# AsyncFlow-Sim/AsyncFlow

Hardware: AMD Instinct MI355X
Metric: simulated request-events/sec (2-server LB scenario, 10k replicas/GPU) (higher is better)
Workload: dtype f64

## Files before the change

### asyncflow_amd/_abi.py

```python

from __future__ import annotations

import ctypes as C

AF_ABI_VERSION = 7

MAX_REQUEST_CAPACITY = 65535
MAX_FIFO_CAPACITY = 1 << 20
COMM_ID_BYTES = 128
AF_OK = 0
AF_ERR_INVALID = -1
AF_ERR_NO_DEVICE = -2
DEVICE_PLAN_ONLY = -1
AF_ERR_HIP = -3
AF_ERR_CAPACITY = -4
AF_ERR_ABI = -5

DIST_CODES = {"poisson": 0, "normal": 1, "log_normal": 2, "exponential": 3, "uniform": 4}
NODE_CLIENT, NODE_LB, NODE_SERVER = 0, 1, 2
LB_CODES = {"round_robin": 0, "least_connection": 1}
STEP_CPU, STEP_IO = 0, 1
METRIC_BITS = {
    "ready_queue_len": 1,
    "event_loop_io_sleep": 2,
# ... 162 lines not shown
        ("flow_fallback", C.c_uint32),
        ("flow_fallback_tie", C.c_uint32),
        ("flow_fallback_list", C.c_uint32),
        ("flow_fallback_ring", C.c_uint32),
        ("flow_fallback_ram", C.c_uint32),
        ("flow_retried", C.c_uint32),
        ("flow_to_next_event", C.c_uint32),
        ("flow_list_entries", C.c_uint32),
        ("flow_ring_rows", C.c_uint32),
        ("flow_lds_bytes", C.c_uint32),
        ("jit_fallbacks", C.c_uint32),
        ("gather_ms", C.c_double),
        ("pregen_group", C.c_uint32),
        ("summary_overlapped", C.c_uint32),
        ("summary_beside_ms", C.c_double),
    ]


FLOW_RING_IN_HBM = 0xFFFFFFFF


class AfSummary(C.Structure):
    _fields_ = [
        ("n_scenarios", C.c_uint32),
        ("rps_buckets", C.c_uint32),
        ("hist_bins", C.c_uint32),
        ("hist_max", C.c_double),
        ("stats", C.c_void_p),
        ("rps", C.c_void_p),
        ("hist", C.c_void_p),
# ... 164 lines not shown
```

### asyncflow_amd/csrc/af_pregen.hpp

```cpp
#pragma once

#include <stdint.h>

#include "af_core.hpp"

namespace afp {

constexpr uint32_t kBatch = 8u;
constexpr uint32_t kRound = 8u;
constexpr uint32_t kChunk = kBatch * kRound;

AF_HD double unit_variate(uint64_t seed, uint32_t idx) {
    const af::U4 r = af::draw_block(seed, af::STREAM_GENERATOR, idx, 0u);
    double u = af::u53(r.x, r.y);
    if (u < 1e-15) u = 1e-15;
    return -af::af_log_unit(1.0 - u);
}

AF_HD double refine_rcp(double d, double r0) {
    const double e0 = __builtin_fma(-d, r0, 1.0);
    const double r1 = __builtin_fma(r0, e0, r0);
    const double e1 = __builtin_fma(-d, r1, 1.0);
    return __builtin_fma(r1, e1, r1);
}
// ... 131 lines not shown
    double total_time, users_mean, users_sigma, rpm, window_s;
    uint32_t users_dist, n_scen, n_draw;
    uint32_t stride;
    uint32_t group;
    const uint64_t* seeds;
    const uint32_t* scen_map;
    uint32_t n_ovr;
    const uint32_t* ovr_param;
    const uint32_t* ovr_index;
    const double* ovr_values;
    uint32_t ovr_stride;
    double* out;
    uint32_t* pre_flags;
};

#if defined(__HIPCC__)
__device__ __forceinline__ double arrival_param(const ArrivalArgs& a, uint32_t param, uint32_t scen, double dflt) {
    for (uint32_t k = 0; k < a.n_ovr; ++k)
        if (a.ovr_param[k] == param && a.ovr_index[k] == 0u) dflt = a.ovr_values[(size_t)k * a.ovr_stride + scen];
    return dflt;
}
__device__ __noinline__ double users_draw_call(uint32_t dist, double mean, double sigma, uint64_t seed, uint32_t idx) {
    return users_draw(dist, mean, sigma, seed, idx);
}

#if !defined(AF_PREGEN_PRODUCERS)
#define AF_PREGEN_PRODUCERS 15
#endif
constexpr uint32_t kProducers = AF_PREGEN_PRODUCERS;
constexpr uint32_t kGroupThreads = 64u * (1u + kProducers);
constexpr uint32_t kIdle = 0xFFFFFFFFu;
typedef double d2_t __attribute__((ext_vector_type(2)));
struct GroupLds {
    double in[2][64][kChunk + 2u];
    double sums[2][64][kChunk + 1u];
    uint64_t seed[64];
    uint32_t d0[64];
    uint32_t sums_k[2][64], sums_n[2][64];
    uint32_t k_final[64];
    uint32_t run[2];
    uint32_t window[2];
};
static_assert(kChunk == 64u, "group_produce / group_store: one wave, one scenario per pass");
__device__ __forceinline__ void group_produce(GroupLds& M, uint32_t buf, uint32_t round, uint32_t n_here, uint32_t ptid) {
    const uint32_t j = ptid & 63u;
    for (uint32_t s = (uint32_t)__builtin_amdgcn_readfirstlane((int)(ptid >> 6)); s < n_here; s += kProducers) {
        const uint32_t d0 = (uint32_t)__builtin_amdgcn_readfirstlane((int)M.d0[s]);
        if (d0 == kIdle) continue;
        const uint32_t lo = (uint32_t)__builtin_amdgcn_readfirstlane((int)(uint32_t)M.seed[s]);
        const uint32_t hi = (uint32_t)__builtin_amdgcn_readfirstlane((int)(uint32_t)(M.seed[s] >> 32));
        M.in[buf][s][j] = unit_variate(((uint64_t)hi << 32) | lo, d0 + round * kChunk + j);
    }
}
__device__ __forceinline__ void group_store(const GroupLds& M, uint32_t buf, double* rows, uint32_t stride, uint32_t n_here,
                                            uint32_t ptid) {
    const uint32_t j = ptid & 63u;
    for (uint32_t s = (uint32_t)__builtin_amdgcn_readfirstlane((int)(ptid >> 6)); s < n_here; s += kProducers) {
        const uint32_t n = (uint32_t)__builtin_amdgcn_readfirstlane((int)M.sums_n[buf][s]);
        const uint32_t k = (uint32_t)__builtin_amdgcn_readfirstlane((int)M.sums_k[buf][s]);
        if (j < n) rows[(size_t)s * stride + k + j] = M.sums[buf][s][j];
    }
}
template <bool FAST_DIV>
__device__ __forceinline__ void group_chain_round(Lane& L, GroupLds& M, uint32_t buf, uint32_t lane, double T, uint32_t n_draw) {
    const uint32_t k0 = L.k;
    d2_t cur[kBatch / 2u], nxt[kBatch / 2u];
#pragma unroll
    for (uint32_t j = 0u; j < kBatch; j += 2u) cur[j / 2u] = *(const d2_t*)&M.in[buf][lane][j];
#pragma unroll
    for (uint32_t st = 0u; st < kRound; ++st) {
        if (st + 1u < kRound) {
#pragma unroll
            for (uint32_t j = 0u; j < kBatch; j += 2u) nxt[j / 2u] = *(const d2_t*)&M.in[buf][lane][(st + 1u) * kBatch + j];
        }
        double e[kBatch], G[kBatch], S[kBatch];
#pragma unroll
        for (uint32_t j = 0u; j < kBatch; j += 2u) {
            e[j] = cur[j / 2u].x;
            e[j + 1u] = cur[j / 2u].y;
        }
        lane_sums<FAST_DIV>(L, e, G, S);
        if (L.state == LANE_RUN) {
            double* o = &M.sums[buf][lane][L.k - k0];
#pragma unroll
            for (uint32_t j = 0u; j < kBatch; ++j) o[j] = S[j];
            if (lane_usual(L, G, T, n_draw)) lane_commit(L, G, S);
            else lane_slow(L, G, S, T, n_draw, nullptr, true);
        }
#pragma unroll
        for (uint32_t j = 0u; j < kBatch / 2u; ++j) cur[j] = nxt[j];
    }
    M.sums_k[buf][lane] = k0;
    M.sums_n[buf][lane] = L.k - k0;
    if (L.state != LANE_RUN) M.d0[lane] = kIdle;
}
__global__ void __launch_bounds__(kGroupThreads) af_arrival_groups(const ArrivalArgs a) {
    extern __shared__ __attribute__((aligned(16))) unsigned char group_smem[];
    GroupLds& M = *reinterpret_cast<GroupLds*>(group_smem);
    const uint32_t tid = threadIdx.x, lane = tid & 63u;
    const bool chain = tid < 64u;
    const uint32_t ptid = tid - 64u;
    const uint32_t slot0 = blockIdx.x * a.group;
    const uint32_t n_here = a.n_scen - slot0 < a.group ? a.n_scen - slot0 : a.group;
    const double T = a.total_time;
    double* rows = a.out + (size_t)slot0 * a.stride;
    const bool valid = chain && lane < n_here;
    const uint32_t slot = slot0 + (valid ? lane : 0u);
    const uint32_t scen = a.scen_map ? a.scen_map[slot] : slot;
    const uint64_t seed = a.seeds[scen];
    double users_mean = 0.0, users_sigma = 0.0, window_s = 0.0, rps_per_user = 0.0;
    Lane L;
    lane_init(L);
    L.state = LANE_DONE;
    if (chain) {
        users_mean = arrival_param(a, af::PARAM_GEN_USERS_MEAN, scen, a.users_mean);
        users_sigma = arrival_param(a, af::PARAM_GEN_USERS_SIGMA, scen, a.users_sigma);
        window_s = arrival_param(a, af::PARAM_GEN_WINDOW, scen, a.window_s);
        rps_per_user = arrival_param(a, af::PARAM_GEN_RPM_MEAN, scen, a.rpm) / 60.0;
        if (valid) L.state = LANE_WAIT;
        M.seed[lane] = seed;
        __builtin_amdgcn_s_setprio(3);
    }
    for (uint32_t w = 0u;; ++w) {
        if (chain) {
            if (L.state == LANE_WAIT)
                window_start(L, T, window_s, rps_per_user,
                             [&](uint32_t idx) { return users_draw_call(a.users_dist, users_mean, users_sigma, seed, idx); });
            M.d0[lane] = L.state == LANE_RUN ? L.draws : kIdle;
            const bool any_run = __any(L.state == LANE_RUN), any_left = __any(L.state != LANE_DONE);
            if (lane == 0u) M.window[w & 1u] = any_run ? 2u : any_left ? 1u : 0u;
        }
        __syncthreads();
        const uint32_t what = M.window[w & 1u];
        if (what == 0u) break;
        if (what == 1u) continue;
        if (!chain) group_produce(M, 0u, 0u, n_here, ptid);
        const bool fast = chain ? !__any(L.state == LANE_RUN && !L.fast_div) : true;
        __syncthreads();
        uint32_t r = 0u;
        for (;;) {
            const uint32_t b = r & 1u;
            if (chain) {
                if (fast) group_chain_round<true>(L, M, b, lane, T, a.n_draw);
                else group_chain_round<false>(L, M, b, lane, T, a.n_draw);
                const bool any_run = __any(L.state == LANE_RUN);
                if (lane == 0u) M.run[b] = any_run ? 1u : 0u;
            } else {
                group_produce(M, b ^ 1u, r + 1u, n_here, ptid);
                if (r > 0u) group_store(M, b ^ 1u, rows, a.stride, n_here, ptid);
            }
            __syncthreads();
            ++r;
            if (M.run[b] == 0u) break;
        }
        if (!chain) group_store(M, (r - 1u) & 1u, rows, a.stride, n_here, ptid);
    }
    if (chain) {
        M.k_final[lane] = L.k;
        if (valid) a.pre_flags[slot] = L.flags;
    }
    __syncthreads();
    for (uint32_t s = 0u; s < n_here; ++s) {
        double* o = rows + (size_t)s * a.stride;
        for (uint32_t i = M.k_final[s] + tid; i < a.n_draw; i += kGroupThreads) o[i] = af::AF_INF;
    }
}
#endif


}
```

### asyncflow_amd/csrc/engine.hip

```cpp
#include <hip/hip_runtime.h>
#include <dlfcn.h>

#include <algorithm>
#include <chrono>
#include <cmath>
#include <cstdio>
#include <cstring>
#include <string>
#include <vector>

#include "../../include/asyncflow_hip.h"
#include "af_core.hpp"
#include "af_flow_host.hpp"
#include "af_plan_pack.hpp"
#include "af_pregen.hpp"
#include "af_summary.hpp"
#include "af_pooled.hpp"
#include "af_series_windows.hpp"
#include "af_windowed.hpp"
#include "af_quantiles.hpp"

#define LDS_AS __attribute__((address_space(3)))

namespace {
// ... 245 lines not shown
        v += dpp<0x111, 0xF>(v);
        v += dpp<0x112, 0xF>(v);
        v += dpp<0x114, 0xF>(v);
        v += dpp<0x118, 0xF>(v);
        v += dpp<0x142, 0xA>(v);
        v += dpp<0x143, 0xC>(v);
        return v;
    }
    static __device__ __forceinline__ uint32_t mbcnt(uint64_t m) {
        return __builtin_amdgcn_mbcnt_hi((uint32_t)(m >> 32), __builtin_amdgcn_mbcnt_lo((uint32_t)m, 0u));
    }
    static __device__ __forceinline__ unsigned long long clock() { return __builtin_amdgcn_s_memtime(); }
};

constexpr uint32_t kDoneWords = 16u;
static __device__ __forceinline__ void signal_scenario_done(const uint32_t* counter_block, uint32_t sc) {
    if (counter_block == nullptr) return;
    const uint64_t* sig = reinterpret_cast<const uint64_t*>(counter_block + kDoneWords);
    uint32_t* flags = reinterpret_cast<uint32_t*>(sig[0]);
    if (flags != nullptr) WaveHip::signal_done(flags + sc, reinterpret_cast<uint32_t*>(sig[1]));
}

#ifndef AF_FLOW_WPE
#define AF_FLOW_WPE 4
#endif
#endif
#ifndef AF_JIT
template <uint32_t IPL, uint32_t FEAT>
__global__ void __launch_bounds__(64) __attribute__((amdgpu_waves_per_eu((FEAT & aff::FEAT_GENSRV) ? 3 : AF_FLOW_WPE))) af_flow_kernel(const aff::FlowArgs a) {
    extern __shared__ __attribute__((aligned(16))) unsigned char smem[];
// ... 280 lines not shown
        for (uint32_t i = k + l; i < a.n_draw; i += G) out[i] = af::AF_INF;
        if (l == 0u) a.pre_flags[slot] = flags;
    }
}


static uint32_t pregen_group_width(uint32_t n) {
    uint32_t group = (n + 255u) / 256u < 64u ? (n + 255u) / 256u : 64u;
    if (const char* env = std::getenv("AF_PREGEN_GROUP")) {
        const int v = std::atoi(env);
        if (v >= 1 && v <= 64) group = (uint32_t)v;
    }
    return group;
}

static int launch_pregen_arrivals(const KArgs& a, uint32_t n, uint32_t stride, bool uniform_load, hipStream_t stream,
                                  bool grouped = false, uint32_t* group_out = nullptr) {
    if (grouped) {
        afp::ArrivalArgs g{};
        g.total_time = a.total_time;
        g.users_mean = a.gen_users_mean;
        g.users_sigma = a.gen_users_sigma;
        g.rpm = a.gen_rpm_mean;
        g.window_s = a.gen_window_s;
        g.users_dist = a.gen_users_dist;
        g.n_scen = n;
        g.n_draw = a.n_draw;
        g.stride = stride;
        g.group = pregen_group_width(n);
        if (group_out) *group_out = g.group;
        g.seeds = a.seeds;
        g.scen_map = a.scen_map;
        g.n_ovr = a.n_ovr;
        g.ovr_param = a.ovr_param;
        g.ovr_index = a.ovr_index;
        g.ovr_values = a.ovr_values;
        g.ovr_stride = a.ovr_stride;
        g.out = a.draws;
        g.pre_flags = a.pre_flags;
        if (hipFuncSetAttribute(reinterpret_cast<const void*>(afp::af_arrival_groups), hipFuncAttributeMaxDynamicSharedMemorySize,
                                (int)sizeof(afp::GroupLds)) != hipSuccess)
            return 1;
        hipLaunchKernelGGL(afp::af_arrival_groups, dim3((n + g.group - 1u) / g.group), dim3(afp::kGroupThreads),
                           sizeof(afp::GroupLds), stream, g);
        return 0;
    }
    double best = 1e300;
    uint32_t best_s = 4u;
    for (uint32_t s : {4u, 5u, 8u}) {
        const double waves = std::ceil((double)n / (double)s);
        if (s != 4u && (!uniform_load || waves / 1024.0 < 1.9)) continue;
        const double cost = std::ceil(waves / 1024.0) * (4.06 * (double)s + 8.0);
        if (cost < best - 1e-9) {
            best = cost;
            best_s = s;
        }
    }
    bool rows = true;
    if (const char* env = std::getenv("AF_PREGEN_SCEN_PER_WAVE")) {
        const uint32_t v = (uint32_t)std::atoi(env);
// ... 131 lines not shown
    double* d_draws = nullptr;
    size_t draws_cap = 0;
    uint32_t* d_pre_flags = nullptr;
    size_t pre_flags_cap = 0;
    uint64_t* d_tie = nullptr;
    size_t tie_cap = 0;
    uint32_t* d_n_shared = nullptr;
    uint32_t* d_map = nullptr;
    size_t map_cap = 0;
    uint32_t* d_order = nullptr;
    size_t order_cap = 0;
    const af_summary_t* fused_sum = nullptr;
    const af_outputs_t* fused_out = nullptr;
    hipStream_t stream2 = nullptr;
    hipEvent_t ev_s0 = nullptr, ev_s1 = nullptr;
    bool fused_done = false;
    uint32_t* d_done_flags = nullptr;
    size_t done_flags_cap = 0;
    uint32_t* h_done_count = nullptr;
    uint32_t* d_done_count = nullptr;
    uint32_t* d_retry = nullptr;
    size_t retry_cap = 0;
    unsigned char* d_pool = nullptr;
    size_t pool_cap = 0;
    int wait_value_ok = -1;
    uint64_t done_ptrs[2] = {0, 0};
    bool shared_instants_likely = false;
    hipModule_t jit_module = nullptr;
    hipFunction_t jit_lean = nullptr, jit_order3 = nullptr, jit_order2 = nullptr;
    std::string jit_spec;
// ... 874 lines not shown
    };
    a.n_draw = n_draw;
    a.n_shared = e->d_n_shared;
    a.scen_map = nullptr;
    a.draw_slot = nullptr;
    a.draws_by_lane = 0u;

    double ms_pregen = 0.0, ms_kernel = 0.0, ms_flow = 0.0;
    uint32_t kl = 0, waves = 0, lds_bytes = 0, n_chunks = 0, n_rerun = 0, n_jit = 0, n_jit_miss = 0;
    uint32_t fused_first = 0u;
    uint32_t fb_total[5] = {0, 0, 0, 0, 0}, flow_scen = 0;
    uint32_t flow_retried = 0, flow_to_next = 0;
    size_t draw_bytes = 0;
    uint32_t pregen_group = 0;
    bool lds_state = false;

    aff::FlowLayout& FL = FP.FL;
    aff::FlowLayout& FL2 = FP.FL2;
    const bool flow_big = FP.big;
    const uint32_t flow_lds = FP.lds;

    const size_t tie_words = a.L.tie_words;
    const bool hetero_load = (mask & ((1u << AF_PARAM_GEN_USERS_MEAN) | (1u << AF_PARAM_GEN_RPM_MEAN))) != 0u;
    auto launch_des = [&](uint32_t count, bool faithful) -> int {
        choose_lanes(e, count, a.blob_bytes, bytes_per_lane, kl, lds_state);
        uint32_t klog = 0;
        while ((1u << klog) < kl) ++klog;
        a.n_scen = count;
        const uint64_t state_per_wave = bytes_per_lane * kl;
        waves = (count + kl - 1) / kl;
// ... 153 lines not shown
        a.pre_flags = e->d_arr_flags;
        const char* pregen_mode = std::getenv("AF_PREGEN_MODE");
        const bool force_groups = pregen_mode && std::strcmp(pregen_mode, "groups") == 0;
        const bool force_rows = pregen_mode && std::strcmp(pregen_mode, "rows") == 0;
        const bool grouped = !force_rows && a.gen_window_s > 0.0 &&
                             (force_groups || (!(mask & (1u << AF_PARAM_GEN_WINDOW)) && nc >= 3072u &&
                                               (double)n_draw * a.gen_window_s >= 512.0 * a.total_time &&
                                               (!hetero_load || load_spread_suits_groups(e, sweep, lo, nc))));
        const bool ordered = hetero_load && std::getenv("AF_FLOW_ORDER_OFF") == nullptr;
        if (ordered) {
            std::vector<uint32_t> order = heaviest_first(e, sweep, lo, nc);
            if (int rc = grow((void**)&e->d_order, e->order_cap, (size_t)nc * 4u)) return rc;
            HIP_TRY(hipMemcpyAsync(e->d_order, order.data(), (size_t)nc * 4u, hipMemcpyHostToDevice, e->stream));
            HIP_TRY(hipStreamSynchronize(e->stream));
        }
        HIP_TRY(hipEventRecord(e->ev2, e->stream));
        if (launch_pregen_arrivals(a, nc, n_draw, !hetero_load, e->stream, grouped, &pregen_group)) return fail(AF_ERR_HIP, "af_arrival_groups: LDS attribute");
        HIP_TRY(hipGetLastError());
        HIP_TRY(hipEventRecord(e->ev3, e->stream));
        aff::FlowArgs f = e->fargs;
        f.L = FL;
        f.n_scen = nc;
        f.seeds = a.seeds;
        f.n_ovr = a.n_ovr;
        f.ovr_param = a.ovr_param;
        f.ovr_index = a.ovr_index;
        f.ovr_values = a.ovr_values;
        f.ovr_stride = a.ovr_stride;
        f.arrivals = e->d_arr;
        f.n_draw = n_draw;
        f.pre_flags = e->d_arr_flags;
        if (ordered) f.scen_map = e->d_order;
        f.clock = a.clock;
        f.clock_cap = a.clock_cap;
// ... 16 lines not shown
        }
        {
            const uint32_t flow_lds_launch = spread_lds_bytes(flow_lds);
            void* kargs[] = {&f};
            const bool jit = e->flow_jit_fn != nullptr && flow_lds_launch <= 64u * 1024u &&
                             flow_jit_spec_string(e, FP, out, sweep->n_overrides != 0u) == e->flow_jit_spec;
            if (e->flow_jit_fn != nullptr && !jit) n_jit_miss += 1u;
            if (std::getenv("AF_DEBUG")) std::fprintf(stderr, "[af] flow jit spec: %s\n", flow_jit_spec_string(e, FP, out, sweep->n_overrides != 0u).c_str());
            if (std::getenv("AF_DEBUG"))
                std::fprintf(stderr, "[af] flow launch: %u scenarios, %u list entries%s, %u ring rows, %u B LDS per wave, af_flow_kernel<%u, %#x>%s%s\n", nc,
                             FL.cap, flow_big ? " (long-list instantiation)" : "", FL.ring_rows, flow_lds, FP.ipl, FP.feat,
                             FP.lean ? (FP.far ? ", lean instantiation with far edges" : ", lean instantiation") : "", jit ? ", plan-specialised" : "");
            const void* fn = jit ? nullptr : flow_kernel_for(FP.ipl, FP.feat);
            if (!jit && fn == nullptr) return fail(AF_ERR_INVALID, "no stage-parallel instantiation for this launch");
            if (!jit && flow_lds_launch > 48u * 1024u) HIP_TRY(hipFuncSetAttribute(fn, hipFuncAttributeMaxDynamicSharedMemorySize, (int)flow_lds_launch));
            uint32_t gate = 0u;
            if (e->fused_sum != nullptr && lo == 0u && nc == n && d_prof == nullptr) {
                if (e->wait_value_ok < 0) {
                    int v = 0;
                    if (hipDeviceGetAttribute(&v, hipDeviceAttributeCanUseStreamWaitValue, e->device) != hipSuccess) { (void)hipGetLastError(); v = 0; }
                    e->wait_value_ok = v;
                }
                int per_cu = 0;
                hipDeviceProp_t prop;
                HIP_TRY(hipGetDeviceProperties(&prop, e->device));
                if (jit) HIP_TRY(hipModuleOccupancyMaxActiveBlocksPerMultiprocessor(&per_cu, e->flow_jit_fn, (int)kWave, flow_lds_launch));
                else HIP_TRY(hipOccupancyMaxActiveBlocksPerMultiprocessor(&per_cu, fn, (int)kWave, flow_lds_launch));
                const uint32_t resident = (uint32_t)(per_cu > 0 ? per_cu : 0) * (uint32_t)prop.multiProcessorCount;
                const uint32_t rem = resident ? nc % resident : 0u;
                if (e->wait_value_ok > 0 && resident != 0u && nc > resident && nc <= 6u * resident && rem != 0u && rem * 4u <= resident * 3u) gate = nc - rem;
                if (std::getenv("AF_DEBUG")) std::fprintf(stderr, "[af] analyzer beside the last round: %u resident waves, gate at %u of %u scenarios\n", resident, gate, nc);
            }
            if (gate != 0u) {
                if (e->stream2 == nullptr) {
                    HIP_TRY(hipStreamCreateWithFlags(&e->stream2, hipStreamNonBlocking));
                    HIP_TRY(hipEventCreate(&e->ev_s0));
                    HIP_TRY(hipEventCreate(&e->ev_s1));
                    HIP_TRY(hipHostMalloc((void**)&e->h_done_count, 64, hipHostMallocCoherent | hipHostMallocMapped));
                    HIP_TRY(hipHostGetDevicePointer((void**)&e->d_done_count, e->h_done_count, 0));
                }
                if (int rc = grow((void**)&e->d_done_flags, e->done_flags_cap, (size_t)nc * 4u)) return rc;
                if (int rc = grow((void**)&e->d_retry, e->retry_cap, 2u * ((size_t)nc + 1u) * 4u)) return rc;
                *e->h_done_count = 0u;
                HIP_TRY(hipMemsetAsync(e->d_done_flags, 0, (size_t)nc * 4u, e->stream));
                HIP_TRY(hipMemsetAsync(e->d_retry, 0, 2u * ((size_t)nc + 1u) * 4u, e->stream));
                e->done_ptrs[0] = reinterpret_cast<uint64_t>(e->d_done_flags);
                e->done_ptrs[1] = reinterpret_cast<uint64_t>(e->d_done_count);
                HIP_TRY(hipMemcpyAsync(e->d_fb + kDoneWords, e->done_ptrs, 16u, hipMemcpyHostToDevice, e->stream));
            }
            f.n_scen = nc;
            if (jit) {
                HIP_TRY(hipModuleLaunchKernel(e->flow_jit_fn, nc, 1, 1, kWave, 1, 1, flow_lds_launch, e->stream, kargs, nullptr));
                n_jit += 1u;
            } else {
                HIP_TRY(hipLaunchKernel(fn, dim3(nc), dim3(kWave), kargs, flow_lds_launch, e->stream));
            }
            if (gate != 0u) {
                auto release_side = [&]() { *e->h_done_count = 0xFFFFFFFFu; };
                hipError_t err = hipStreamWaitValue32(e->stream2, e->d_done_count, gate, hipStreamWaitValueGte, 0xFFFFFFFFu);
                if (err == hipSuccess) err = hipEventRecord(e->ev_s0, e->stream2);
                int rc = AF_OK;
                if (err == hipSuccess) rc = launch_summary_kernels(e, e->fused_out, e->fused_sum, 0u, nc, e->stream2, e->d_done_flags, e->d_retry, nullptr, 0u);
                if (err == hipSuccess && rc == AF_OK) err = hipEventRecord(e->ev_s1, e->stream2);
                if (err != hipSuccess || rc != AF_OK) {
                    release_side();
                    (void)hipStreamSynchronize(e->stream);
                    (void)hipStreamSynchronize(e->stream2);
                    if (rc != AF_OK) return rc;
                    HIP_TRY(err);
                }
// ... 26 lines not shown
                for (uint32_t k = 0; k < aff::kProfSections; ++k) acc[k] += (double)hp[(size_t)i * aff::kProfSections + k];
            for (uint32_t k = 0; k < aff::kProfSections; ++k)
                if (!names[k] || std::strncmp(names[k], "COUNT", 5) != 0) total += acc[k];
            if (FILE* fp = std::fopen(prof_path, "a")) {
                std::fprintf(fp, "af_flow_kernel<%u, %#x> sections, %u waves, mean cycles per wave %.0f:\n", FP.ipl, FP.feat, nc, total / nc);
                for (uint32_t k = 0; k < aff::kProfSections; ++k)
                    if (names[k]) std::fprintf(fp, "  %-28s %6.2f %%  %12.0f cycles per wave\n", names[k], 100.0 * acc[k] / total, acc[k] / nc);
                std::fclose(fp);
            }
        }
        float ms_p = 0.f, ms_f = 0.f;
        HIP_TRY(hipEventElapsedTime(&ms_p, e->ev2, e->ev3));
        HIP_TRY(hipEventElapsedTime(&ms_f, e->ev3, e->ev4));
        ms_pregen += ms_p;
        ms_flow += ms_f;
        flow_scen += nc;
        for (int k = 0; k < 5; ++k) fb_total[k] += fb[k];
        if (fb[0] > 0u) {
            std::vector<uint32_t> cnt_host((size_t)nc * AF_CNT_SLOTS);
            HIP_TRY(hipMemcpy(cnt_host.data(), a.counts, cnt_host.size() * 4u, hipMemcpyDeviceToHost));
            std::vector<uint32_t> retry, rest;
            for (uint32_t i = 0; i < nc; ++i) {
                const uint32_t fl = cnt_host[(size_t)i * AF_CNT_SLOTS + AF_CNT_FLAGS];
                if (!(fl & aff::FLAG_FLOW_FALLBACK)) continue;
                if ((fl & (aff::FLOW_WHY_RAM | aff::FLOW_WHY_GEN_TIE)) || (flow_big && !FP.gen_compact)) rest.push_back(i);
                else retry.push_back(i);
            }
            if (!retry.empty()) {
                if (int rc = grow((void**)&e->d_map, e->map_cap, retry.size() * 4u)) return rc;
                HIP_TRY(hipMemcpyAsync(e->d_map, retry.data(), retry.size() * 4u, hipMemcpyHostToDevice, e->stream));
// ... 58 lines not shown
    e->stats.flow_kernel_ms = ms_flow;
    e->stats.flow_scenarios = flow_scen;
    e->stats.flow_fallback = fb_total[0];
    e->stats.flow_fallback_tie = fb_total[1];
    e->stats.flow_fallback_list = fb_total[2];
    e->stats.flow_fallback_ring = fb_total[3];
    e->stats.flow_fallback_ram = fb_total[4];
    e->stats.flow_retried = flow_retried;
    e->stats.flow_to_next_event = flow_to_next;
    e->stats.flow_list_entries = flow_scen ? FL.cap : 0u;
    e->stats.flow_ring_rows = flow_scen ? FL.ring_rows : 0u;
    e->stats.flow_lds_bytes = flow_lds;
    e->stats.jit_fallbacks = n_jit_miss;
    e->stats.pregen_group = pregen_group;
    e->stats.pregen_ms = ms_pregen;
    e->stats.h2d_ms = ms_h2d;
    e->stats.draw_bytes = draw_bytes;
    e->stats.state_bytes_per_scenario = bytes_per_lane;
    e->stats.state_in_lds = lds_state ? 1u : 0u;
    e->stats.lds_bytes_per_wave = lds_bytes;
    e->stats.waves = waves;
    e->stats.lanes_per_wave = kl;
    e->stats.chunks = n_chunks;
    e->stats.shared_instant_scenarios = n_rerun;
    e->stats.specialised_launches = n_jit;
    e->stats.request_capacity = e->request_capacity;
    e->stats.fifo_capacity = e->fifo_capacity;
    return AF_OK;
}

// ... 831 lines not shown
        delete e;
        return;
    }
    (void)hipSetDevice(e->device);
    if (e->d_blob) (void)hipFree(e->d_blob);
    if (e->d_state) (void)hipFree(e->d_state);
    if (e->d_sweep) (void)hipFree(e->d_sweep);
    if (e->ev0) (void)hipEventDestroy(e->ev0);
    if (e->ev1) (void)hipEventDestroy(e->ev1);
    if (e->ev2) (void)hipEventDestroy(e->ev2);
    if (e->ev3) (void)hipEventDestroy(e->ev3);
    if (e->ev4) (void)hipEventDestroy(e->ev4);
    if (e->ev_s0) (void)hipEventDestroy(e->ev_s0);
    if (e->ev_s1) (void)hipEventDestroy(e->ev_s1);
    if (e->stream2) (void)hipStreamDestroy(e->stream2);
    if (e->d_done_flags) (void)hipFree(e->d_done_flags);
    if (e->d_retry) (void)hipFree(e->d_retry);
    if (e->d_pool) (void)hipFree(e->d_pool);
    if (e->h_done_count) (void)hipHostFree(e->h_done_count);
    if (e->d_draws) (void)hipFree(e->d_draws);
    if (e->d_pre_flags) (void)hipFree(e->d_pre_flags);
    if (e->d_tie) (void)hipFree(e->d_tie);
    if (e->d_n_shared) (void)hipFree(e->d_n_shared);
    if (e->d_map) (void)hipFree(e->d_map);
    if (e->d_order) (void)hipFree(e->d_order);
    if (e->d_tick) (void)hipFree(e->d_tick);
    if (e->d_arr) (void)hipFree(e->d_arr);
    if (e->d_arr_flags) (void)hipFree(e->d_arr_flags);
    if (e->d_fb) (void)hipFree(e->d_fb);
    if (e->d_slot) (void)hipFree(e->d_slot);
// ... 207 lines not shown
```

### include/asyncflow_hip.h

```cpp
#ifndef ASYNCFLOW_HIP_H
#define ASYNCFLOW_HIP_H

#include <stddef.h>
#include <stdint.h>

#ifdef __cplusplus
extern "C" {
#endif

#define AF_ABI_VERSION 7

enum af_status {
    AF_OK = 0,
    AF_ERR_INVALID = -1,
    AF_ERR_NO_DEVICE = -2,
    AF_ERR_HIP = -3,
    AF_ERR_CAPACITY = -4,
    AF_ERR_ABI = -5
};

enum af_dist {
    AF_DIST_POISSON = 0,
    AF_DIST_NORMAL = 1,
    AF_DIST_LOG_NORMAL = 2,
// ... 169 lines not shown
    uint32_t flow_fallback;
    uint32_t flow_fallback_tie;
    uint32_t flow_fallback_list;
    uint32_t flow_fallback_ring;
    uint32_t flow_fallback_ram;
    uint32_t flow_retried;
    uint32_t flow_to_next_event;
    uint32_t flow_list_entries;
    uint32_t flow_ring_rows;
    uint32_t flow_lds_bytes;
    uint32_t jit_fallbacks;
    double gather_ms;
    uint32_t pregen_group;
    uint32_t summary_overlapped;
    double summary_beside_ms;
} af_stats_t;

typedef struct af_engine af_engine_t;

#define AF_DEVICE_PLAN_ONLY (-1)
int af_engine_create(const af_plan_t* plan, int device, const af_engine_options_t* opts,
                     af_engine_t** out);
int af_engine_jit_spec(af_engine_t* engine, const af_sweep_t* sweep, const af_outputs_t* out, char* buf, size_t cap);
int af_engine_set_kernels(af_engine_t* engine, const char* spec, const void* image, size_t size);

typedef struct af_summary_t {
    uint32_t n_scenarios;
    uint32_t rps_buckets;
    uint32_t hist_bins;
    double hist_max;
// ... 102 lines not shown
```

Baseline: 123.6 billion.

## Split pregen and flow launches across two streams to overlap the partial round

When the flow kernel's scenario count leaves a partial last round of resident waves, the scenarios in that remainder are now pre-generated and simulated first on the main stream. The remaining scenarios have their arrivals pre-generated on a second stream, using a smaller producer count, while that first part runs. The grouped arrival kernel is templated on producer count, and its LDS layout becomes dynamically sized by group width, so a lighter variant can run beside the flow kernel. The aim is to fill idle CUs in the tail and hide pre-generation time, at the cost of an extra stream, events, an identity map buffer, and possible contention between the concurrent kernels.

```diff
diff --git a/asyncflow_amd/_abi.py b/asyncflow_amd/_abi.py
--- a/asyncflow_amd/_abi.py
+++ b/asyncflow_amd/_abi.py
@@ -200,6 +200,9 @@
         ("pregen_group", C.c_uint32),
         ("summary_overlapped", C.c_uint32),
         ("summary_beside_ms", C.c_double),
+        ("pregen_beside_ms", C.c_double),
+        ("flow_split_first", C.c_uint32),
+        ("flow_resident", C.c_uint32),
     ]
 
 
diff --git a/asyncflow_amd/csrc/af_pregen.hpp b/asyncflow_amd/csrc/af_pregen.hpp
--- a/asyncflow_amd/csrc/af_pregen.hpp
+++ b/asyncflow_amd/csrc/af_pregen.hpp
@@ -169,6 +169,102 @@
     uint32_t* pre_flags;
 };
 
+constexpr uint32_t kIdle = 0xFFFFFFFFu;
+constexpr uint32_t kInPitch = kChunk + 2u;
+constexpr uint32_t kSumsPitch = kChunk + 1u;
+constexpr uint32_t kTailInf = 64u;
+typedef double d2_t __attribute__((vector_size(16)));
+struct GroupLds {
+    unsigned char* base;
+    uint32_t group;
+    AF_HD static uint32_t off_sums(uint32_t g) { return 2u * g * kInPitch * 8u; }
+    AF_HD static uint32_t off_seed(uint32_t g) { return off_sums(g) + 2u * g * kSumsPitch * 8u; }
+    AF_HD static uint32_t off_words(uint32_t g) { return off_seed(g) + g * 8u; }
+    AF_HD static uint32_t bytes(uint32_t g) { return (off_words(g) + (6u * g + 4u) * 4u + 15u) & ~15u; }
+    AF_HD double* in(uint32_t buf, uint32_t s) const { return reinterpret_cast<double*>(base) + (size_t)(buf * group + s) * kInPitch; }
+    AF_HD double* sums(uint32_t buf, uint32_t s) const {
+        return reinterpret_cast<double*>(base + off_sums(group)) + (size_t)(buf * group + s) * kSumsPitch;
+    }
+    AF_HD uint64_t* seed() const { return reinterpret_cast<uint64_t*>(base + off_seed(group)); }
+    AF_HD uint32_t* words() const { return reinterpret_cast<uint32_t*>(base + off_words(group)); }
+    AF_HD uint32_t* d0() const { return words(); }
+    AF_HD uint32_t* sums_k(uint32_t buf) const { return words() + (1u + buf) * group; }
+    AF_HD uint32_t* sums_n(uint32_t buf) const { return words() + (3u + buf) * group; }
+    AF_HD uint32_t* k_final() const { return words() + 5u * group; }
+    AF_HD uint32_t* run() const { return words() + 6u * group; }
+    AF_HD uint32_t* window() const { return words() + 6u * group + 2u; }
+};
+#if defined(__HIP_DEVICE_COMPILE__)
+#define AFP_UNIFORM(x) ((uint32_t)__builtin_amdgcn_readfirstlane((int)(x)))
+#else
+#define AFP_UNIFORM(x) ((uint32_t)(x))
+#endif
+static_assert(kChunk == 64u, "group_produce / group_store: one wave, one scenario per pass");
+AF_HD void group_produce(const GroupLds& M, uint32_t buf, uint32_t round, uint32_t n_here, uint32_t ptid, uint32_t producers) {
+    const uint32_t j = ptid & 63u;
+    for (uint32_t s = AFP_UNIFORM(ptid >> 6); s < n_here; s += producers) {
+        const uint32_t d0 = AFP_UNIFORM(M.d0()[s]);
+        if (d0 == kIdle) continue;
+        const uint32_t lo = AFP_UNIFORM((uint32_t)M.seed()[s]);
+        const uint32_t hi = AFP_UNIFORM((uint32_t)(M.seed()[s] >> 32));
+        M.in(buf, s)[j] = unit_variate(((uint64_t)hi << 32) | lo, d0 + round * kChunk + j);
+    }
+}
+AF_HD void group_store(const GroupLds& M, uint32_t buf, double* rows, uint32_t stride, uint32_t n_here, uint32_t ptid,
+                       uint32_t producers) {
+    const uint32_t j = ptid & 63u;
+    for (uint32_t s = AFP_UNIFORM(ptid >> 6); s < n_here; s += producers) {
+        const uint32_t n = AFP_UNIFORM(M.sums_n(buf)[s]);
+        const uint32_t k = AFP_UNIFORM(M.sums_k(buf)[s]);
+        if (j < n) rows[(size_t)s * stride + k + j] = M.sums(buf, s)[j];
+    }
+}
+template <bool FAST_DIV>
+AF_HD void group_chain_round(Lane& L, const GroupLds& M, uint32_t buf, uint32_t lane, double T, uint32_t n_draw) {
+    const uint32_t k0 = L.k;
+    const double* in = M.in(buf, lane);
+    double* sums = M.sums(buf, lane);
+    d2_t cur[kBatch / 2u], nxt[kBatch / 2u];
+#pragma unroll
+    for (uint32_t j = 0u; j < kBatch; j += 2u) cur[j / 2u] = *(const d2_t*)&in[j];
+#pragma unroll
+    for (uint32_t st = 0u; st < kRound; ++st) {
+        if (st + 1u < kRound) {
+#pragma unroll
+            for (uint32_t j = 0u; j < kBatch; j += 2u) nxt[j / 2u] = *(const d2_t*)&in[(st + 1u) * kBatch + j];
+        }
+        double e[kBatch], G[kBatch], S[kBatch];
+#pragma unroll
+        for (uint32_t j = 0u; j < kBatch; j += 2u) {
+            e[j] = cur[j / 2u][0];
+            e[j + 1u] = cur[j / 2u][1];
+        }
+        lane_sums<FAST_DIV>(L, e, G, S);
+        if (L.state == LANE_RUN) {
+            double* o = &sums[L.k - k0];
+#pragma unroll
+            for (uint32_t j = 0u; j < kBatch; ++j) o[j] = S[j];
+            if (lane_usual(L, G, T, n_draw)) lane_commit(L, G, S);
+            else lane_slow(L, G, S, T, n_draw, nullptr, true);
+        }
+        if (st + 1u < kRound) {
+#pragma unroll
+            for (uint32_t j = 0u; j < kBatch / 2u; ++j) cur[j] = nxt[j];
+        }
+    }
+    M.sums_k(buf)[lane] = k0;
+    M.sums_n(buf)[lane] = L.k - k0;
+    if (L.state != LANE_RUN) M.d0()[lane] = kIdle;
+}
+AF_HD void group_fill_tail(const GroupLds& M, double* rows, uint32_t stride, uint32_t n_draw, uint32_t n_here, uint32_t tid,
+                           uint32_t threads) {
+    const uint32_t j = tid & 63u;
+    for (uint32_t s = tid >> 6; s < n_here; s += threads >> 6) {
+        const uint32_t i = M.k_final()[s] + j;
+        if (j < kTailInf && i < n_draw) rows[(size_t)s * stride + i] = af::AF_INF;
+    }
+}
+
 #if defined(__HIPCC__)
 __device__ __forceinline__ double arrival_param(const ArrivalArgs& a, uint32_t param, uint32_t scen, double dflt) {
     for (uint32_t k = 0; k < a.n_ovr; ++k)
@@ -183,75 +279,13 @@
 #define AF_PREGEN_PRODUCERS 15
 #endif
 constexpr uint32_t kProducers = AF_PREGEN_PRODUCERS;
-constexpr uint32_t kGroupThreads = 64u * (1u + kProducers);
-constexpr uint32_t kIdle = 0xFFFFFFFFu;
-typedef double d2_t __attribute__((ext_vector_type(2)));
-struct GroupLds {
-    double in[2][64][kChunk + 2u];
-    double sums[2][64][kChunk + 1u];
-    uint64_t seed[64];
-    uint32_t d0[64];
-    uint32_t sums_k[2][64], sums_n[2][64];
-    uint32_t k_final[64];
-    uint32_t run[2];
-    uint32_t window[2];
-};
-static_assert(kChunk == 64u, "group_produce / group_store: one wave, one scenario per pass");
-__device__ __forceinline__ void group_produce(GroupLds& M, uint32_t buf, uint32_t round, uint32_t n_here, uint32_t ptid) {
-    const uint32_t j = ptid & 63u;
-    for (uint32_t s = (uint32_t)__builtin_amdgcn_readfirstlane((int)(ptid >> 6)); s < n_here; s += kProducers) {
-        const uint32_t d0 = (uint32_t)__builtin_amdgcn_readfirstlane((int)M.d0[s]);
-        if (d0 == kIdle) continue;
-        const uint32_t lo = (uint32_t)__builtin_amdgcn_readfirstlane((int)(uint32_t)M.seed[s]);
-        const uint32_t hi = (uint32_t)__builtin_amdgcn_readfirstlane((int)(uint32_t)(M.seed[s] >> 32));
-        M.in[buf][s][j] = unit_variate(((uint64_t)hi << 32) | lo, d0 + round * kChunk + j);
-    }
-}
-__device__ __forceinline__ void group_store(const GroupLds& M, uint32_t buf, double* rows, uint32_t stride, uint32_t n_here,
-                                            uint32_t ptid) {
-    const uint32_t j = ptid & 63u;
-    for (uint32_t s = (uint32_t)__builtin_amdgcn_readfirstlane((int)(ptid >> 6)); s < n_here; s += kProducers) {
-        const uint32_t n = (uint32_t)__builtin_amdgcn_readfirstlane((int)M.sums_n[buf][s]);
-        const uint32_t k = (uint32_t)__builtin_amdgcn_readfirstlane((int)M.sums_k[buf][s]);
-        if (j < n) rows[(size_t)s * stride + k + j] = M.sums[buf][s][j];
-    }
-}
-template <bool FAST_DIV>
-__device__ __forceinline__ void group_chain_round(Lane& L, GroupLds& M, uint32_t buf, uint32_t lane, double T, uint32_t n_draw) {
-    const uint32_t k0 = L.k;
-    d2_t cur[kBatch / 2u], nxt[kBatch / 2u];
-#pragma unroll
-    for (uint32_t j = 0u; j < kBatch; j += 2u) cur[j / 2u] = *(const d2_t*)&M.in[buf][lane][j];
-#pragma unroll
-    for (uint32_t st = 0u; st < kRound; ++st) {
-        if (st + 1u < kRound) {
-#pragma unroll
-            for (uint32_t j = 0u; j < kBatch; j += 2u) nxt[j / 2u] = *(const d2_t*)&M.in[buf][lane][(st + 1u) * kBatch + j];
-        }
-        double e[kBatch], G[kBatch], S[kBatch];
-#pragma unroll
-        for (uint32_t j = 0u; j < kBatch; j += 2u) {
-            e[j] = cur[j / 2u].x;
-            e[j + 1u] = cur[j / 2u].y;
-        }
-        lane_sums<FAST_DIV>(L, e, G, S);
-        if (L.state == LANE_RUN) {
-            double* o = &M.sums[buf][lane][L.k - k0];
-#pragma unroll
-            for (uint32_t j = 0u; j < kBatch; ++j) o[j] = S[j];
-            if (lane_usual(L, G, T, n_draw)) lane_commit(L, G, S);
-            else lane_slow(L, G, S, T, n_draw, nullptr, true);
-        }
-#pragma unroll
-        for (uint32_t j = 0u; j < kBatch / 2u; ++j) cur[j] = nxt[j];
-    }
-    M.sums_k[buf][lane] = k0;
-    M.sums_n[buf][lane] = L.k - k0;
-    if (L.state != LANE_RUN) M.d0[lane] = kIdle;
-}
-__global__ void __launch_bounds__(kGroupThreads) af_arrival_groups(const ArrivalArgs a) {
+constexpr uint32_t kProducersBeside = 7u;
+template <uint32_t P>
+__global__ void __launch_bounds__(64u * (1u + P)) __attribute__((amdgpu_waves_per_eu(4))) af_arrival_groups(const ArrivalArgs a) {
+    static_assert(P >= 1u && P <= 15u, "a workgroup is at most 16 waves");
+    constexpr uint32_t kGroupThreads = 64u * (1u + P);
     extern __shared__ __attribute__((aligned(16))) unsigned char group_smem[];
-    GroupLds& M = *reinterpret_cast<GroupLds*>(group_smem);
+    const GroupLds M{group_smem, a.group};
     const uint32_t tid = threadIdx.x, lane = tid & 63u;
     const bool chain = tid < 64u;
     const uint32_t ptid = tid - 64u;
@@ -272,8 +306,10 @@
         users_sigma = arrival_param(a, af::PARAM_GEN_USERS_SIGMA, scen, a.users_sigma);
         window_s = arrival_param(a, af::PARAM_GEN_WINDOW, scen, a.window_s);
         rps_per_user = arrival_param(a, af::PARAM_GEN_RPM_MEAN, scen, a.rpm) / 60.0;
-        if (valid) L.state = LANE_WAIT;
-        M.seed[lane] = seed;
+        if (valid) {
+            L.state = LANE_WAIT;
+            M.seed()[lane] = seed;
+        }
         __builtin_amdgcn_s_setprio(3);
     }
     for (uint32_t w = 0u;; ++w) {
@@ -281,44 +317,43 @@
             if (L.state == LANE_WAIT)
                 window_start(L, T, window_s, rps_per_user,
                              [&](uint32_t idx) { return users_draw_call(a.users_dist, users_mean, users_sigma, seed, idx); });
-            M.d0[lane] = L.state == LANE_RUN ? L.draws : kIdle;
+            if (valid) M.d0()[lane] = L.state == LANE_RUN ? L.draws : kIdle;
             const bool any_run = __any(L.state == LANE_RUN), any_left = __any(L.state != LANE_DONE);
-            if (lane == 0u) M.window[w & 1u] = any_run ? 2u : any_left ? 1u : 0u;
+            if (lane == 0u) M.window()[w & 1u] = any_run ? 2u : any_left ? 1u : 0u;
         }
         __syncthreads();
-        const uint32_t what = M.window[w & 1u];
+        const uint32_t what = M.window()[w & 1u];
         if (what == 0u) break;
         if (what == 1u) continue;
-        if (!chain) group_produce(M, 0u, 0u, n_here, ptid);
+        if (!chain) group_produce(M, 0u, 0u, n_here, ptid, P);
         const bool fast = chain ? !__any(L.state == LANE_RUN && !L.fast_div) : true;
         __syncthreads();
         uint32_t r = 0u;
         for (;;) {
             const uint32_t b = r & 1u;
             if (chain) {
-                if (fast) group_chain_round<true>(L, M, b, lane, T, a.n_draw);
-                else group_chain_round<false>(L, M, b, lane, T, a.n_draw);
+                if (valid) {
+                    if (fast) group_chain_round<true>(L, M, b, lane, T, a.n_draw);
+                    else group_chain_round<false>(L, M, b, lane, T, a.n_draw);
+                }
                 const bool any_run = __any(L.state == LANE_RUN);
-                if (lane == 0u) M.run[b] = any_run ? 1u : 0u;
+                if (lane == 0u) M.run()[b] = any_run ? 1u : 0u;
             } else {
-                group_produce(M, b ^ 1u, r + 1u, n_here, ptid);
-                if (r > 0u) group_store(M, b ^ 1u, rows, a.stride, n_here, ptid);
+                group_produce(M, b ^ 1u, r + 1u, n_here, ptid, P);
+                if (r > 0u) group_store(M, b ^ 1u, rows, a.stride, n_here, ptid, P);
             }
             __syncthreads();
             ++r;
-            if (M.run[b] == 0u) break;
-        }
-        if (!chain) group_store(M, (r - 1u) & 1u, rows, a.stride, n_here, ptid);
-    }
-    if (chain) {
-        M.k_final[lane] = L.k;
-        if (valid) a.pre_flags[slot] = L.flags;
+            if (M.run()[b] == 0u) break;
+        }
+        if (!chain) group_store(M, (r - 1u) & 1u, rows, a.stride, n_here, ptid, P);
+    }
+    if (valid) {
+        M.k_final()[lane] = L.k;
+        a.pre_flags[slot] = L.flags;
     }
     __syncthreads();
-    for (uint32_t s = 0u; s < n_here; ++s) {
-        double* o = rows + (size_t)s * a.stride;
-        for (uint32_t i = M.k_final[s] + tid; i < a.n_draw; i += kGroupThreads) o[i] = af::AF_INF;
-    }
+    group_fill_tail(M, rows, a.stride, a.n_draw, n_here, tid, kGroupThreads);
 }
 #endif
 
diff --git a/asyncflow_amd/csrc/engine.hip b/asyncflow_amd/csrc/engine.hip
--- a/asyncflow_amd/csrc/engine.hip
+++ b/asyncflow_amd/csrc/engine.hip
@@ -283,6 +283,7 @@
 };
 
 constexpr uint32_t kDoneWords = 16u;
+constexpr bool kFlowSplitDefault = true;
 static __device__ __forceinline__ void signal_scenario_done(const uint32_t* counter_block, uint32_t sc) {
     if (counter_block == nullptr) return;
     const uint64_t* sig = reinterpret_cast<const uint64_t*>(counter_block + kDoneWords);
@@ -593,8 +594,17 @@
     return group;
 }
 
+template <uint32_t P>
+static int launch_arrival_groups(const afp::ArrivalArgs& g, hipStream_t stream) {
+    const uint32_t lds = afp::GroupLds::bytes(g.group);
+    if (hipFuncSetAttribute(reinterpret_cast<const void*>(afp::af_arrival_groups<P>), hipFuncAttributeMaxDynamicSharedMemorySize, (int)lds) != hipSuccess)
+        return 1;
+    hipLaunchKernelGGL(afp::af_arrival_groups<P>, dim3((g.n_scen + g.group - 1u) / g.group), dim3(64u * (1u + P)), lds, stream, g);
+    return 0;
+}
+
 static int launch_pregen_arrivals(const KArgs& a, uint32_t n, uint32_t stride, bool uniform_load, hipStream_t stream,
-                                  bool grouped = false, uint32_t* group_out = nullptr) {
+                                  bool grouped = false, uint32_t* group_out = nullptr, uint32_t base = 0u, bool beside = false) {
     if (grouped) {
         afp::ArrivalArgs g{};
         g.total_time = a.total_time;
@@ -608,21 +618,17 @@
         g.stride = stride;
         g.group = pregen_group_width(n);
         if (group_out) *group_out = g.group;
-        g.seeds = a.seeds;
+        g.seeds = a.seeds + base;
         g.scen_map = a.scen_map;
         g.n_ovr = a.n_ovr;
         g.ovr_param = a.ovr_param;
         g.ovr_index = a.ovr_index;
-        g.ovr_values = a.ovr_values;
+        g.ovr_values = a.ovr_values + base;
         g.ovr_stride = a.ovr_stride;
-        g.out = a.draws;
-        g.pre_flags = a.pre_flags;
-        if (hipFuncSetAttribute(reinterpret_cast<const void*>(afp::af_arrival_groups), hipFuncAttributeMaxDynamicSharedMemorySize,
-                                (int)sizeof(afp::GroupLds)) != hipSuccess)
-            return 1;
-        hipLaunchKernelGGL(afp::af_arrival_groups, dim3((n + g.group - 1u) / g.group), dim3(afp::kGroupThreads),
-                           sizeof(afp::GroupLds), stream, g);
-        return 0;
+        g.out = a.draws + (size_t)base * stride;
+        g.pre_flags = a.pre_flags + base;
+        if (beside && afp::kProducers > afp::kProducersBeside) return launch_arrival_groups<afp::kProducersBeside>(g, stream);
+        return launch_arrival_groups<afp::kProducers>(g, stream);
     }
     double best = 1e300;
     uint32_t best_s = 4u;
@@ -784,6 +790,11 @@
     const af_outputs_t* fused_out = nullptr;
     hipStream_t stream2 = nullptr;
     hipEvent_t ev_s0 = nullptr, ev_s1 = nullptr;
+    hipStream_t stream3 = nullptr;
+    hipEvent_t ev_a0 = nullptr, ev_a1 = nullptr, ev_a2 = nullptr;
+    uint32_t* d_ident = nullptr;
+    uint32_t ident_n = 0;
+    int n_cu = -1;
     bool fused_done = false;
     uint32_t* d_done_flags = nullptr;
     size_t done_flags_cap = 0;
@@ -1688,6 +1699,9 @@
     size_t draw_bytes = 0;
     uint32_t pregen_group = 0;
     bool lds_state = false;
+    bool split_used = false;
+    double ms_pregen_beside = 0.0;
+    uint32_t split_first = 0u, flow_resident = 0u;
 
     aff::FlowLayout& FL = FP.FL;
     aff::FlowLayout& FL2 = FP.FL2;
@@ -1871,10 +1885,6 @@
             HIP_TRY(hipMemcpyAsync(e->d_order, order.data(), (size_t)nc * 4u, hipMemcpyHostToDevice, e->stream));
             HIP_TRY(hipStreamSynchronize(e->stream));
         }
-        HIP_TRY(hipEventRecord(e->ev2, e->stream));
-        if (launch_pregen_arrivals(a, nc, n_draw, !hetero_load, e->stream, grouped, &pregen_group)) return fail(AF_ERR_HIP, "af_arrival_groups: LDS attribute");
-        HIP_TRY(hipGetLastError());
-        HIP_TRY(hipEventRecord(e->ev3, e->stream));
         aff::FlowArgs f = e->fargs;
         f.L = FL;
         f.n_scen = nc;
@@ -1921,6 +1931,17 @@
             const void* fn = jit ? nullptr : flow_kernel_for(FP.ipl, FP.feat);
             if (!jit && fn == nullptr) return fail(AF_ERR_INVALID, "no stage-parallel instantiation for this launch");
             if (!jit && flow_lds_launch > 48u * 1024u) HIP_TRY(hipFuncSetAttribute(fn, hipFuncAttributeMaxDynamicSharedMemorySize, (int)flow_lds_launch));
+            if (e->n_cu < 0) {
+                hipDeviceProp_t prop;
+                HIP_TRY(hipGetDeviceProperties(&prop, e->device));
+                e->n_cu = prop.multiProcessorCount;
+            }
+            int per_cu = 0;
+            if (jit) HIP_TRY(hipModuleOccupancyMaxActiveBlocksPerMultiprocessor(&per_cu, e->flow_jit_fn, (int)kWave, flow_lds_launch));
+            else HIP_TRY(hipOccupancyMaxActiveBlocksPerMultiprocessor(&per_cu, fn, (int)kWave, flow_lds_launch));
+            const uint32_t resident = (uint32_t)(per_cu > 0 ? per_cu : 0) * (uint32_t)e->n_cu;
+            const uint32_t rem = resident ? nc % resident : 0u;
+            flow_resident = resident;
             uint32_t gate = 0u;
             if (e->fused_sum != nullptr && lo == 0u && nc == n && d_prof == nullptr) {
                 if (e->wait_value_ok < 0) {
@@ -1928,16 +1949,13 @@
                     if (hipDeviceGetAttribute(&v, hipDeviceAttributeCanUseStreamWaitValue, e->device) != hipSuccess) { (void)hipGetLastError(); v = 0; }
                     e->wait_value_ok = v;
                 }
-                int per_cu = 0;
-                hipDeviceProp_t prop;
-                HIP_TRY(hipGetDeviceProperties(&prop, e->device));
-                if (jit) HIP_TRY(hipModuleOccupancyMaxActiveBlocksPerMultiprocessor(&per_cu, e->flow_jit_fn, (int)kWave, flow_lds_launch));
-                else HIP_TRY(hipOccupancyMaxActiveBlocksPerMultiprocessor(&per_cu, fn, (int)kWave, flow_lds_launch));
-                const uint32_t resident = (uint32_t)(per_cu > 0 ? per_cu : 0) * (uint32_t)prop.multiProcessorCount;
-                const uint32_t rem = resident ? nc % resident : 0u;
                 if (e->wait_value_ok > 0 && resident != 0u && nc > resident && nc <= 6u * resident && rem != 0u && rem * 4u <= resident * 3u) gate = nc - rem;
                 if (std::getenv("AF_DEBUG")) std::fprintf(stderr, "[af] analyzer beside the last round: %u resident waves, gate at %u of %u scenarios\n", resident, gate, nc);
             }
+            const char* split_env = std::getenv("AF_FLOW_SPLIT");
+            const bool split = (split_env != nullptr ? std::atoi(split_env) != 0 : kFlowSplitDefault) && std::getenv("ROCPROF_COUNTER_COLLECTION") == nullptr &&
+                               grouped && !ordered && d_prof == nullptr && resident != 0u && nc > resident && nc <= 6u * resident &&
+                               rem != 0u && rem * 8u >= resident;
             if (gate != 0u) {
                 if (e->stream2 == nullptr) {
                     HIP_TRY(hipStreamCreateWithFlags(&e->stream2, hipStreamNonBlocking));
@@ -1955,12 +1973,64 @@
                 e->done_ptrs[1] = reinterpret_cast<uint64_t>(e->d_done_count);
                 HIP_TRY(hipMemcpyAsync(e->d_fb + kDoneWords, e->done_ptrs, 16u, hipMemcpyHostToDevice, e->stream));
             }
-            f.n_scen = nc;
-            if (jit) {
-                HIP_TRY(hipModuleLaunchKernel(e->flow_jit_fn, nc, 1, 1, kWave, 1, 1, flow_lds_launch, e->stream, kargs, nullptr));
-                n_jit += 1u;
+            auto launch_flow = [&](uint32_t first, uint32_t count, const uint32_t* map, hipStream_t st) -> hipError_t {
+                (void)first;
+                f.n_scen = count;
+                f.scen_map = map;
+                if (jit) {
+                    n_jit += 1u;
+                    return hipModuleLaunchKernel(e->flow_jit_fn, count, 1, 1, kWave, 1, 1, flow_lds_launch, st, kargs, nullptr);
+                }
+                return hipLaunchKernel(fn, dim3(count), dim3(kWave), kargs, flow_lds_launch, st);
+            };
+            if (!split) {
+                HIP_TRY(hipEventRecord(e->ev2, e->stream));
+                if (launch_pregen_arrivals(a, nc, n_draw, !hetero_load, e->stream, grouped, &pregen_group)) return fail(AF_ERR_HIP, "af_arrival_groups: LDS attribute");
+                HIP_TRY(hipGetLastError());
+                HIP_TRY(hipEventRecord(e->ev3, e->stream));
+                HIP_TRY(launch_flow(0u, nc, ordered ? e->d_order : nullptr, e->stream));
             } else {
-                HIP_TRY(hipLaunchKernel(fn, dim3(nc), dim3(kWave), kargs, flow_lds_launch, e->stream));
+                if (e->stream3 == nullptr) {
+                    HIP_TRY(hipStreamCreateWithFlags(&e->stream3, hipStreamNonBlocking));
+                    HIP_TRY(hipEventCreate(&e->ev_a0));
+                    HIP_TRY(hipEventCreate(&e->ev_a1));
+                    HIP_TRY(hipEventCreate(&e->ev_a2));
+                }
+                if (nc > e->ident_n) {
+                    std::vector<uint32_t> ident(nc);
+                    for (uint32_t i = 0; i < nc; ++i) ident[i] = i;
+                    if (e->d_ident) HIP_TRY(hipFree(e->d_ident));
+                    e->d_ident = nullptr;
+                    e->ident_n = 0u;
+                    HIP_TRY(hipMalloc((void**)&e->d_ident, (size_t)nc * 4u));
+                    HIP_TRY(hipMemcpy(e->d_ident, ident.data(), (size_t)nc * 4u, hipMemcpyHostToDevice));
+                    e->ident_n = nc;
+                }
+                const uint32_t n_a = nc - rem;
+                if (std::getenv("AF_DEBUG")) std::fprintf(stderr, "[af] split launch: %u scenarios first (the partial round of %u slots), %u beside and behind them\n", rem, resident, n_a);
+                HIP_TRY(hipEventRecord(e->ev2, e->stream));
+                HIP_TRY(hipStreamWaitEvent(e->stream3, e->ev2, 0));
+                hipError_t err = hipSuccess;
+                int lds_fail = launch_pregen_arrivals(a, rem, n_draw, !hetero_load, e->stream, true, nullptr, 0u, false);
+                if (!lds_fail) err = hipGetLastError();
+                if (!lds_fail && err == hipSuccess) err = hipEventRecord(e->ev3, e->stream);
+                if (!lds_fail && err == hipSuccess) err = hipEventRecord(e->ev_a0, e->stream3);
+                if (!lds_fail && err == hipSuccess) lds_fail = launch_pregen_arrivals(a, n_a, n_draw, !hetero_load, e->stream3, true, &pregen_group, rem, true);
+                if (!lds_fail && err == hipSuccess) err = hipGetLastError();
+                if (!lds_fail && err == hipSuccess) err = hipEventRecord(e->ev_a1, e->stream3);
+                if (!lds_fail && err == hipSuccess) err = launch_flow(0u, rem, e->d_ident, e->stream);
+                if (!lds_fail && err == hipSuccess) err = launch_flow(rem, n_a, e->d_ident + rem, e->stream3);
+                if (!lds_fail && err == hipSuccess) err = hipEventRecord(e->ev_a2, e->stream3);
+                if (!lds_fail && err == hipSuccess) err = hipStreamWaitEvent(e->stream, e->ev_a2, 0);
+                if (lds_fail || err != hipSuccess) {
+                    if (gate != 0u) *e->h_done_count = 0xFFFFFFFFu;
+                    (void)hipStreamSynchronize(e->stream3);
+                    (void)hipStreamSynchronize(e->stream);
+                    if (lds_fail) return fail(AF_ERR_HIP, "af_arrival_groups: LDS attribute");
+                    HIP_TRY(err);
+                }
+                split_used = true;
+                split_first = rem;
             }
             if (gate != 0u) {
                 auto release_side = [&]() { *e->h_done_count = 0xFFFFFFFFu; };
@@ -2017,6 +2087,15 @@
         HIP_TRY(hipEventElapsedTime(&ms_f, e->ev3, e->ev4));
         ms_pregen += ms_p;
         ms_flow += ms_f;
+        if (split_used) {
+            float ms_pa = 0.f, ms_fa = 0.f;
+            HIP_TRY(hipEventElapsedTime(&ms_pa, e->ev_a0, e->ev_a1));
+            HIP_TRY(hipEventElapsedTime(&ms_fa, e->ev_a1, e->ev_a2));
+            ms_pregen_beside += ms_pa;
+            if (std::getenv("AF_DEBUG"))
+                std::fprintf(stderr, "[af] split launch: pre-generation %.3f ms alone, %.3f ms beside the first part; kernel %.3f ms, its second part %.3f ms\n", ms_p, ms_pa, ms_f, ms_fa);
+            split_used = false;
+        }
         flow_scen += nc;
         for (int k = 0; k < 5; ++k) fb_total[k] += fb[k];
         if (fb[0] > 0u) {
@@ -2105,6 +2184,9 @@
     e->stats.jit_fallbacks = n_jit_miss;
     e->stats.pregen_group = pregen_group;
     e->stats.pregen_ms = ms_pregen;
+    e->stats.pregen_beside_ms = ms_pregen_beside;
+    e->stats.flow_split_first = split_first;
+    e->stats.flow_resident = flow_resident;
     e->stats.h2d_ms = ms_h2d;
     e->stats.draw_bytes = draw_bytes;
     e->stats.state_bytes_per_scenario = bytes_per_lane;
@@ -2966,6 +3048,11 @@
     if (e->ev_s0) (void)hipEventDestroy(e->ev_s0);
     if (e->ev_s1) (void)hipEventDestroy(e->ev_s1);
     if (e->stream2) (void)hipStreamDestroy(e->stream2);
+    if (e->ev_a0) (void)hipEventDestroy(e->ev_a0);
+    if (e->ev_a1) (void)hipEventDestroy(e->ev_a1);
+    if (e->ev_a2) (void)hipEventDestroy(e->ev_a2);
+    if (e->stream3) (void)hipStreamDestroy(e->stream3);
+    if (e->d_ident) (void)hipFree(e->d_ident);
     if (e->d_done_flags) (void)hipFree(e->d_done_flags);
     if (e->d_retry) (void)hipFree(e->d_retry);
     if (e->d_pool) (void)hipFree(e->d_pool);
diff --git a/include/asyncflow_hip.h b/include/asyncflow_hip.h
--- a/include/asyncflow_hip.h
+++ b/include/asyncflow_hip.h
@@ -207,6 +207,9 @@
     uint32_t pregen_group;
     uint32_t summary_overlapped;
     double summary_beside_ms;
+    double pregen_beside_ms;
+    uint32_t flow_split_first;
+    uint32_t flow_resident;
 } af_stats_t;
 
 typedef struct af_engine af_engine_t;
```

Result: slower. 116.3 billion (-5.9%).
